# maxjaritz/mvpnet

Hardware: AMD Instinct MI355X
Metric: chunks/sec (8192 pts, 3x160x120 views) fwd+bwd (higher is better)
Workload: dtype f32; 1 GPU; configs[2]: MVPNet lifting (unproject + pixel k-NN + gather) + FeatureAggregation + PN2SSG full train step (fwd+loss+bwd+Adam), 2D CNN replaced by a resident 64-ch feature map; cfg=mvpnet_3d_unet_resnet34_pn2ssg.yaml, chunks_per_gpu=32, points=8192, views=3x160x120, feature_channels=64, k=3, parallelism=dp1 (one process per GPU, 1 grad all-reduce/step), launch=eager, cpu_affinity=32 logical cpus of 256 (0 .. 183)

## Files before the change

include/mvp_hip.h:

```cpp
#ifndef MVP_HIP_H_
#define MVP_HIP_H_

#include <stddef.h>
#include <stdint.h>

#ifdef __cplusplus
extern "C" {
#endif

typedef void* mvp_stream_t;

#define MVP_OK 0
#define MVP_EINVAL (-1)
#define MVP_EUNSUPPORTED (-2)
#define MVP_ENULL (-3)

const char* mvp_version(void);
const char* mvp_strerror(int code);

int mvp_set_fps_mode(int mode);

int mvp_fps_f32(const float* points, int64_t B, int64_t N, int64_t D, int64_t M, int64_t* index, mvp_stream_t stream);
int mvp_fps_f64(const double* points, int64_t B, int64_t N, int64_t D, int64_t M, int64_t* index, mvp_stream_t stream);
int mvp_fps_shape_f32(const float* points, int64_t B, int64_t N, int64_t D, int64_t M, int64_t* index, int shape, mvp_stream_t stream);
// ... 291 lines not shown
                             const float* act_mean, const float* act_invstd, const float* act_gamma, const float* act_beta, float* ymax,
                             float* ymin, uint8_t* amax, uint8_t* amin, double* stat, double* partial, float eps, float momentum,
                             float* mean, float* invstd, float* running_mean, float* running_var, int64_t* num_batches_tracked,
                             mvp_stream_t stream);
int mvp_pool_finalize_f32(const float* ymax, const float* ymin, const uint8_t* amax, const uint8_t* amin, const float* mean,
                          const float* invstd, const float* gamma, const float* beta, int64_t G, int64_t C, int relu, float* out,
                          uint8_t* arg, float* ysel, mvp_stream_t stream);
int mvp_pool_backward_stats_f32(const float* dout, const float* out, const float* ysel, const float* mean, const float* invstd,
                                int64_t G, int64_t C, int relu, double* stat, double* partial, mvp_stream_t stream);
int mvp_mlp_input_grad_f32(const float* dY, int64_t R, int64_t Cout, const float* W, int64_t Cin, const float* y_prev,
                           const float* mean, const float* invstd, const float* gamma, const float* beta, float* dZ,
                           double* stat, double* partial, mvp_stream_t stream);
int mvp_mlp_input_grad_dropout_f32(const float* dY, int64_t R, int64_t Cout, const float* W, int64_t Cin, const float* y_prev,
                                   const float* mean, const float* invstd, const float* gamma, const float* beta, float drop_p,
                                   uint64_t drop_seed, float* dZ, double* stat, double* partial, mvp_stream_t stream);

int64_t mvp_mlp_layer_backward_partial_count(int64_t R, int64_t Cp);
int mvp_mlp_layer_backward_f32(const float* G, const float* Yi, const float* mean_i, const float* invstd_i, const float* gamma_i,
                               const double* stat_i, float* dgamma_i, float* dbeta_i, int training, const float* X, int64_t ldx,
                               const float* act_mean, const float* act_invstd, const float* act_gamma, const float* act_beta,
                               const float* W, int64_t ldw, int64_t R, int64_t C, int64_t Cp, float* dW, int64_t lddw, float* dZ,
                               double* stat_prev, double* partial, const float* pool_dout, const float* pool_out,
                               const uint8_t* pool_arg, mvp_stream_t stream);
int mvp_mlp_layer_backward_ws_f32(const float* G, const float* Yi, const float* mean_i, const float* invstd_i, const float* gamma_i,
                               const double* stat_i, float* dgamma_i, float* dbeta_i, int training, const float* X, int64_t ldx,
                               const float* act_mean, const float* act_invstd, const float* act_gamma, const float* act_beta,
                               const float* W, int64_t ldw, int64_t R, int64_t C, int64_t Cp, float* dW, int64_t lddw, float* dZ,
                               double* stat_prev, double* partial, const float* pool_dout, const float* pool_out,
                               const uint8_t* pool_arg, float* workspace, int64_t workspace_floats, mvp_stream_t stream);
int mvp_mlp_layer_backward_wide_p_f32(const float* G, const float* Yi, const float* mean_i, const float* invstd_i, const float* gamma_i,
// ... 83 lines not shown
    num_batches_tracked, int precision, int precision_backward, mvp_stream_t stream);
int mvp_mlp_forward_rel_bn_p_f32(const float* X, int64_t R, int64_t Cin, int64_t ldx, const float* W, int64_t ldw, int64_t Cout,
    const float* rel, const float* wrel, float* Y, double* stat, double* partial, float eps, float momentum, float* mean, float*
    invstd, float* running_mean, float* running_var, int64_t* num_batches_tracked, int precision, int precision_backward,
    mvp_stream_t stream);
int mvp_mlp_forward_pool_p_f32(const float* X, int64_t R, int64_t Cin, int64_t ldx, const float* W, int64_t ldw, int64_t Cout,
    const float* act_mean, const float* act_invstd, const float* act_gamma, const float* act_beta, float* ymax, float* ymin,
    uint8_t* amax, uint8_t* amin, double* stat, double* partial, float eps, float momentum, float* mean, float* invstd, float*
    running_mean, float* running_var, int64_t* num_batches_tracked, int precision, int precision_backward, mvp_stream_t stream);
int mvp_mlp_input_grad_p_f32(const float* dY, int64_t R, int64_t Cout, const float* W, int64_t Cin, const float* y_prev, const
    float* mean, const float* invstd, const float* gamma, const float* beta, float* dZ, double* stat, double* partial, int
    precision, int precision_backward, mvp_stream_t stream);
int mvp_mlp_input_grad_dropout_p_f32(const float* dY, int64_t R, int64_t Cout, const float* W, int64_t Cin, const float* y_prev, const
    float* mean, const float* invstd, const float* gamma, const float* beta, float drop_p, uint64_t drop_seed, float* dZ, double* stat,
    double* partial, int precision, int precision_backward, mvp_stream_t stream);
int mvp_mlp_weight_grad_p_f32(const float* dY, const float* X, int64_t R, int64_t Cout, int64_t Cin, int64_t ldx, const float*
    act_mean, const float* act_invstd, const float* act_gamma, const float* act_beta, float* dW, int64_t lddw, int precision,
    int precision_backward, mvp_stream_t stream);
int mvp_mlp_weight_grad_ws_p_f32(const float* dY, const float* X, int64_t R, int64_t Cout, int64_t Cin, int64_t ldx, const
    float* act_mean, const float* act_invstd, const float* act_gamma, const float* act_beta, float* dW, int64_t lddw, float*
    workspace, int64_t workspace_floats, int precision, int precision_backward, mvp_stream_t stream);
int mvp_mlp_layer_backward_p_f32(const float* G, const float* Yi, const float* mean_i, const float* invstd_i, const float*
    gamma_i, const double* stat_i, float* dgamma_i, float* dbeta_i, int training, const float* X, int64_t ldx, const float*
    act_mean, const float* act_invstd, const float* act_gamma, const float* act_beta, const float* W, int64_t ldw, int64_t R,
    int64_t C, int64_t Cp, float* dW, int64_t lddw, float* dZ, double* stat_prev, double* partial, const float* pool_dout, const
    float* pool_out, const uint8_t* pool_arg, int precision, int precision_backward, mvp_stream_t stream);
int mvp_mlp_layer_backward_ws_p_f32(const float* G, const float* Yi, const float* mean_i, const float* invstd_i, const float*
    gamma_i, const double* stat_i, float* dgamma_i, float* dbeta_i, int training, const float* X, int64_t ldx, const float*
    act_mean, const float* act_invstd, const float* act_gamma, const float* act_beta, const float* W, int64_t ldw, int64_t R,
    int64_t C, int64_t Cp, float* dW, int64_t lddw, float* dZ, double* stat_prev, double* partial, const float* pool_dout, const
// ... 92 lines not shown
```

mvpnet_amd/csrc/mlp.hip:

```cpp
#include "common.h"
#include "stats_reduce.h"
#include "mlp_common.h"
#include "dropout.h"
#include <algorithm>

int mvp_mlp_stream_forward(const float* X, int64_t R, int Cin, int ldx, const float* W, int ldw, int Cout, const float* act_mean,
                           const float* act_invstd, const float* act_gamma, const float* act_beta, const float* bias, float* Y,
                           double* stat, double* partial, int ns, float bn_eps, float bn_momentum, float* bn_mean, float* bn_invstd,
                           float* bn_running_mean, float* bn_running_var, int64_t* bn_num_batches, float* ymax, float* ymin,
                           uint8_t* amax, uint8_t* amin, hipStream_t s);

int g_mlp_terms = 6;
int g_mlp_terms_bwd = 3;
int g_mlp_min_width = 0;
thread_local int tl_mlp_terms = -1;
thread_local int tl_mlp_terms_bwd = -1;
int g_mlp_stream = 1;

namespace {


constexpr int kMT = 256;
constexpr int kBM = 128;

// ... 613 lines not shown
    for (int i = 0; i < 16; ++i) {
      const int co = co0 + wco + (i & 3) + 8 * (i >> 2) + 4 * (lane >> 5);
#ifdef MVP_EXP_DW_STORE
      if (co < Cout && ci < Cin) *(dW + (size_t)co * lddw + ci) = acc[i];
#else
      if (co < Cout && ci < Cin) atomicAdd(dW + (size_t)co * lddw + ci, acc[i]);
#endif
    }
  }
}

template <int TMB, int TNB, int NS, bool FIN = false, bool REL = false>
__global__ __launch_bounds__(kMT) void mlp_dw_bf_kernel(const float* __restrict__ dY, const float* __restrict__ X, int64_t R,
                                                        int Cout, int Cin, int ldx, InAct act, int64_t rows_per_block,
                                                        float* __restrict__ dW, int lddw, float* __restrict__ ws, DyFinish fin = DyFinish{},
                                                        const float* __restrict__ X2 = nullptr, float* __restrict__ dW2 = nullptr) {
  using SP = SplitPairs<NS>;
  constexpr int NRB = REL ? TMB : 0;
  __shared__ float red[2][(TMB * TNB + NRB) * 16 * 64];
  const int tid = threadIdx.x, lane = tid & 63, wave = tid >> 6;
  const int c = lane & 31, g = lane >> 5;
  const int co0 = blockIdx.x * (32 * TMB), ci0 = blockIdx.y * (32 * TNB);
  const int64_t r_begin = (int64_t)blockIdx.z * rows_per_block;
  const int64_t r_end = min(R, r_begin + rows_per_block);
  f32x16 acc[TMB][TNB];
#pragma unroll
  for (int a = 0; a < TMB; ++a)
#pragma unroll
    for (int b = 0; b < TNB; ++b)
#pragma unroll
      for (int i = 0; i < 16; ++i) acc[a][b][i] = 0.f;
// ... 72 lines not shown
      unsigned q[4][NS];
#pragma unroll
      for (int h2 = 0; h2 < 4; ++h2) split_pair<NS>(v[2 * h2], v[2 * h2 + 1], q[h2]);
#pragma unroll
      for (int pc = 0; pc < NS; ++pc) fa[a][pc] = u32x4{q[0][pc], q[1][pc], q[2][pc], q[3][pc]};
    }
#pragma unroll
    for (int b = 0; b < TNB; ++b) {
      float v[8];
#pragma unroll
      for (int p = 0; p < 8; ++p) {
        float x = xn[b][p];
        if (has_act) {
          const float z = ((x - pm[b]) * pi[b]) * pg[b] + pb[b];
          x = z > 0.f ? z : 0.f;
        }
        v[p] = (rok[p] && xok[b]) ? x : 0.f;
      }
      unsigned q[4][NS];
#pragma unroll
      for (int h2 = 0; h2 < 4; ++h2) split_pair<NS>(v[2 * h2], v[2 * h2 + 1], q[h2]);
#pragma unroll
      for (int pc = 0; pc < NS; ++pc) fb[b][pc] = u32x4{q[0][pc], q[1][pc], q[2][pc], q[3][pc]};
    }
    if constexpr (REL) {
      float v[8];
#pragma unroll
      for (int p = 0; p < 8; ++p) v[p] = (rok[p] && c < 4) ? rn[p] : 0.f;
      unsigned q[4][NS];
#pragma unroll
// ... 350 lines not shown
                         rows_per_block, dW, (int)lddw, w);                                                                        \
    else                                                                                                                           \
      hipLaunchKernelGGL((mlp_dw_kernel<M_, N_, false>), grid, dim3(kMT), 0, s, dY, X, R, (int)Cout, (int)Cin, (int)ldx, act,        \
                         rows_per_block, dW, (int)lddw, w);                                                                        \
    if (w)                                                                                                                         \
      hipLaunchKernelGGL((dw_reduce_kernel<(M_) / 32, (N_) / 32>), dim3((unsigned)(tiles * ((M_) / 32) * ((N_) / 32) * 16)), dim3(256), 0, \
                         s, w, (int)splits, (int)grid.x, (int)grid.y, (int)Cout, (int)Cin, dW, (int)lddw);                         \
  } while (0)
  if (TM == 32 && TN == 32) MVP_DW_LAUNCH(32, 32);
  else if (TM == 32) MVP_DW_LAUNCH(32, 64);
  else if (TN == 32) MVP_DW_LAUNCH(64, 32);
  else MVP_DW_LAUNCH(64, 64);
#undef MVP_DW_LAUNCH
  return mvp_launch_status();
}
}

MVP_API int mvp_mlp_weight_grad_f32(const float* dY, const float* X, int64_t R, int64_t Cout, int64_t Cin, int64_t ldx,
                                    const float* act_mean, const float* act_invstd, const float* act_gamma,
                                    const float* act_beta, float* dW, int64_t lddw, mvp_stream_t stream) {
  return weight_grad_impl(dY, X, R, Cout, Cin, ldx, act_mean, act_invstd, act_gamma, act_beta, dW, lddw, nullptr, 0, stream);
}

MVP_API int64_t mvp_mlp_weight_grad_workspace_floats(void) { return (int64_t)1536 * 4096; }
MVP_API int mvp_mlp_weight_grad_ws_f32(const float* dY, const float* X, int64_t R, int64_t Cout, int64_t Cin, int64_t ldx,
                                       const float* act_mean, const float* act_invstd, const float* act_gamma, const float* act_beta,
                                       float* dW, int64_t lddw, float* workspace, int64_t workspace_floats, mvp_stream_t stream) {
  return weight_grad_impl(dY, X, R, Cout, Cin, ldx, act_mean, act_invstd, act_gamma, act_beta, dW, lddw, workspace, workspace_floats, stream);
}

// ... 157 lines not shown
```

mvpnet_amd/csrc/mlp_prec.hip:

```cpp
#include "mlp_common.h"

namespace {
struct PrecisionArg {
  int old_terms, old_bwd;
  bool ok;
  PrecisionArg(int terms, int bwd) : old_terms(tl_mlp_terms), old_bwd(tl_mlp_terms_bwd) {
    ok = (terms == -1 || terms == 0 || terms == 1 || terms == 3 || terms == 6) && (bwd == -1 || bwd == 1 || bwd == 3 || bwd == 6);
    if (ok && terms >= 0) tl_mlp_terms = terms;
    if (ok && bwd >= 0) tl_mlp_terms_bwd = bwd;
  }
  ~PrecisionArg() {
    tl_mlp_terms = old_terms;
    tl_mlp_terms_bwd = old_bwd;
  }
};
}

#define MVP_WITH_PRECISION(call)             \
  PrecisionArg scope(precision, precision_backward); \
  if (!scope.ok) return MVP_EINVAL;          \
  return call

MVP_API int mvp_mlp_forward_p_f32(const float* X, int64_t R, int64_t Cin, int64_t ldx, const float* W, int64_t ldw, int64_t Cout,
                                  const float* act_mean, const float* act_invstd, const float* act_gamma, const float* act_beta,
// ... 22 lines not shown
                                       float momentum, float* mean, float* invstd, float* running_mean, float* running_var,
                                       int64_t* num_batches_tracked, int precision, int precision_backward, mvp_stream_t stream) {
  MVP_WITH_PRECISION(mvp_mlp_forward_pool_f32(X, R, Cin, ldx, W, ldw, Cout, act_mean, act_invstd, act_gamma, act_beta, ymax, ymin, amax, amin, stat,
                                              partial, eps, momentum, mean, invstd, running_mean, running_var, num_batches_tracked, stream));
}
MVP_API int mvp_mlp_input_grad_p_f32(const float* dY, int64_t R, int64_t Cout, const float* W, int64_t Cin, const float* y_prev,
                                     const float* mean, const float* invstd, const float* gamma, const float* beta, float* dZ, double* stat,
                                     double* partial, int precision, int precision_backward, mvp_stream_t stream) {
  MVP_WITH_PRECISION(mvp_mlp_input_grad_f32(dY, R, Cout, W, Cin, y_prev, mean, invstd, gamma, beta, dZ, stat, partial, stream));
}
MVP_API int mvp_mlp_input_grad_dropout_p_f32(const float* dY, int64_t R, int64_t Cout, const float* W, int64_t Cin, const float* y_prev,
                                             const float* mean, const float* invstd, const float* gamma, const float* beta, float drop_p,
                                             uint64_t drop_seed, float* dZ, double* stat, double* partial, int precision, int precision_backward,
                                             mvp_stream_t stream) {
  MVP_WITH_PRECISION(mvp_mlp_input_grad_dropout_f32(dY, R, Cout, W, Cin, y_prev, mean, invstd, gamma, beta, drop_p, drop_seed, dZ, stat, partial, stream));
}
MVP_API int mvp_mlp_weight_grad_p_f32(const float* dY, const float* X, int64_t R, int64_t Cout, int64_t Cin, int64_t ldx,
                                      const float* act_mean, const float* act_invstd, const float* act_gamma, const float* act_beta,
                                      float* dW, int64_t lddw, int precision, int precision_backward, mvp_stream_t stream) {
  MVP_WITH_PRECISION(mvp_mlp_weight_grad_f32(dY, X, R, Cout, Cin, ldx, act_mean, act_invstd, act_gamma, act_beta, dW, lddw, stream));
}
MVP_API int mvp_mlp_weight_grad_ws_p_f32(const float* dY, const float* X, int64_t R, int64_t Cout, int64_t Cin, int64_t ldx,
                                         const float* act_mean, const float* act_invstd, const float* act_gamma, const float* act_beta,
                                         float* dW, int64_t lddw, float* workspace, int64_t workspace_floats, int precision,
                                         int precision_backward, mvp_stream_t stream) {
  MVP_WITH_PRECISION(mvp_mlp_weight_grad_ws_f32(dY, X, R, Cout, Cin, ldx, act_mean, act_invstd, act_gamma, act_beta, dW, lddw, workspace,
                                                workspace_floats, stream));
}
MVP_API int mvp_mlp_layer_backward_p_f32(const float* G, const float* Yi, const float* mean_i, const float* invstd_i, const float* gamma_i,
                                         const double* stat_i, float* dgamma_i, float* dbeta_i, int training, const float* X, int64_t ldx,
// ... 76 lines not shown
```

mvpnet_amd/csrc/mlp_stream.hip:

```cpp
#include "mlp_common.h"
#include "stats_reduce.h"
#include <algorithm>

namespace {

constexpr int kST = 256;
constexpr int kSLd = 36;

struct StreamArgs {
  const float* X;
  int64_t R;
  int Cin, ldx;
  const float* W;
  int ldw, Cout;
  InAct act;
  const float* bias;
  float* Y;
  double* partial;
  double* stat;
  int finalize;
  BnFinalize fin;
  int64_t tiles_per_wg;
  float* ymax;
  float* ymin;
  uint8_t* amax;
  uint8_t* amin;
};

template <int KS, int NB, bool ACT, int NS, bool POOL>
__global__ __launch_bounds__(kST) void mlp_stream_fwd_kernel(StreamArgs p) {
  using SP = SplitPairs<NS>;
  constexpr int kCols = NB * 32;
  constexpr int kWBytes = KS * NS * kCols * 64;
  __shared__ __attribute__((aligned(16))) unsigned char Wl[kWBytes];
  __shared__ __attribute__((aligned(16))) float Ps[4][KS * 32];
  __shared__ __attribute__((aligned(16))) float tiles[4][32 * kSLd];
  __shared__ double sred[2][4][kCols];
  const int tid = threadIdx.x, lane = tid & 63, wave = tid >> 6;
  const int li = lane & 31, lh = lane >> 5;
  const int Cin = p.Cin, Cout = p.Cout;

  for (int t = tid; t < kCols * KS * 8; t += kST) {
    const int co = t % kCols, kqi = t / kCols;
    const int k = 4 * kqi;
    float v[4];
// ... 41 lines not shown
      for (int tt = 0; tt < 4; ++tt) dst[sl][tt] = *reinterpret_cast<const float4*>(xrow + min(32 * sl + 8 * tt + 4 * lh, Cin - 4));
  };
#pragma unroll
  for (int u = 0; u < PF; ++u)
    if (t_begin + wave + 4 * u < t_end) load_a(an[u], t_begin + wave + 4 * u);
  for (int64_t tb = t_begin + wave; tb < t_end; tb += 4 * PF) {
#pragma unroll
   for (int u = 0; u < PF; ++u) {
    const int64_t t = tb + 4 * u;
    if (t >= t_end) break;
    float4 ac[KS][4];
#pragma unroll
    for (int sl = 0; sl < KS; ++sl)
#pragma unroll
      for (int tt = 0; tt < 4; ++tt) ac[sl][tt] = an[u][sl][tt];
    if (t + 4 * PF < t_end) load_a(an[u], t + 4 * PF);
    f32x16 acc[NB];
#pragma unroll
    for (int j = 0; j < NB; ++j)
#pragma unroll
      for (int i = 0; i < 16; ++i) acc[j][i] = 0.f;
#pragma unroll
    for (int sl = 0; sl < KS; ++sl) {
      float v[4][4];
#pragma unroll
      for (int tt = 0; tt < 4; ++tt) {
        v[tt][0] = ac[sl][tt].x; v[tt][1] = ac[sl][tt].y; v[tt][2] = ac[sl][tt].z; v[tt][3] = ac[sl][tt].w;
        if constexpr (ACT) {
          const int k = 32 * sl + 8 * tt + 4 * lh;
          const float4 m4 = *reinterpret_cast<const float4*>(&Ps[0][k]), i4 = *reinterpret_cast<const float4*>(&Ps[1][k]);
          const float4 g4 = *reinterpret_cast<const float4*>(&Ps[2][k]), b4 = *reinterpret_cast<const float4*>(&Ps[3][k]);
          const float pm[4] = {m4.x, m4.y, m4.z, m4.w}, pi[4] = {i4.x, i4.y, i4.z, i4.w};
          const float pg[4] = {g4.x, g4.y, g4.z, g4.w}, pb[4] = {b4.x, b4.y, b4.z, b4.w};
#pragma unroll
          for (int e = 0; e < 4; ++e) {
            const float a = ((v[tt][e] - pm[e]) * pi[e]) * pg[e] + pb[e];
            v[tt][e] = a > 0.f ? a : 0.f;
          }
        }
      }
#pragma unroll
      for (int s = 0; s < 2; ++s) {
        unsigned q0[NS], q1[NS], q2[NS], q3[NS];
        split_pair<NS>(v[2 * s][0], v[2 * s][1], q0);
        split_pair<NS>(v[2 * s][2], v[2 * s][3], q1);
        split_pair<NS>(v[2 * s + 1][0], v[2 * s + 1][1], q2);
        split_pair<NS>(v[2 * s + 1][2], v[2 * s + 1][3], q3);
        u32x4 af[NS];
#pragma unroll
        for (int pc = 0; pc < NS; ++pc) af[pc] = u32x4{q0[pc], q1[pc], q2[pc], q3[pc]};
        constexpr int JG = NB >= 2 ? 2 : 1;
#pragma unroll
// ... 132 lines not shown
    }
  }
}

template <int KS, int NB, int NS>
void launch_stream(const StreamArgs& a, unsigned grid, bool has_act, hipStream_t s) {
  if (a.ymax) {
    if (has_act) hipLaunchKernelGGL((mlp_stream_fwd_kernel<KS, NB, true, NS, true>), dim3(grid), dim3(kST), 0, s, a);
    else hipLaunchKernelGGL((mlp_stream_fwd_kernel<KS, NB, false, NS, true>), dim3(grid), dim3(kST), 0, s, a);
    return;
  }
  if (has_act) hipLaunchKernelGGL((mlp_stream_fwd_kernel<KS, NB, true, NS, false>), dim3(grid), dim3(kST), 0, s, a);
  else hipLaunchKernelGGL((mlp_stream_fwd_kernel<KS, NB, false, NS, false>), dim3(grid), dim3(kST), 0, s, a);
}

}

int mvp_mlp_stream_forward(const float* X, int64_t R, int Cin, int ldx, const float* W, int ldw, int Cout, const float* act_mean,
                           const float* act_invstd, const float* act_gamma, const float* act_beta, const float* bias, float* Y,
                           double* stat, double* partial, int ns, float bn_eps, float bn_momentum, float* bn_mean, float* bn_invstd,
                           float* bn_running_mean, float* bn_running_var, int64_t* bn_num_batches, float* ymax, float* ymin,
                           uint8_t* amax, uint8_t* amin, hipStream_t s) {
  const InAct act{act_mean, act_invstd, act_gamma, act_beta};
  if (ns == 0 || Cin > 128 || Cout > 128 || Cin < 4 || Cout % 4 != 0 || R < 32768 || (stat && !partial)) return MVP_EUNSUPPORTED;
  if (ldx % 4 != 0 || Cin % 4 != 0 || ((uintptr_t)X % 16) != 0 || (!ymax && ((uintptr_t)Y % 16) != 0)) return MVP_EUNSUPPORTED;
  if (ymax && R % 32 != 0) return MVP_EUNSUPPORTED;
  static const bool tail = []() { const char* e = getenv("MVP_STREAM_TAIL"); return !(e && e[0] == '0'); }();
  StreamArgs a{X, R, Cin, ldx, W, ldw, Cout, act, bias, Y, (stat && !tail) ? partial : nullptr, (stat && tail) ? stat : nullptr, bn_mean ? 1 : 0,
               BnFinalize{R, bn_eps, bn_momentum, bn_mean, bn_invstd, bn_running_mean, bn_running_var, bn_num_batches}, 0, ymax, ymin, amax, amin};
  const int64_t ntiles = cdiv(R, 32);
  const int ks = (int)cdiv(Cin, 32), nb = Cout <= 32 ? 1 : Cout <= 64 ? 2 : 4;
  const int64_t lds = (int64_t)ks * ns * nb * 32 * 64;
  const int64_t per_cu = std::max<int64_t>(1, std::min<int64_t>(4, (140 * 1024) / (lds + 24 * 1024)));
  int64_t wgs = std::min<int64_t>(256 * per_cu, std::min<int64_t>(cdiv(R, 128), cdiv(ntiles, 16)));
  wgs = std::max<int64_t>(wgs, 1);
  a.tiles_per_wg = cdiv(cdiv(ntiles, wgs), 4) * 4;
  const unsigned grid = (unsigned)cdiv(ntiles, a.tiles_per_wg);
  const bool has_act = act.mean != nullptr;
#define MVP_STREAM(KS_, NB_)                                                      \
  do {                                                                            \
    if (ns == 1) launch_stream<KS_, NB_, 1>(a, grid, has_act, s);                  \
    else if (ns == 2) launch_stream<KS_, NB_, 2>(a, grid, has_act, s);             \
    else launch_stream<KS_, NB_, 3>(a, grid, has_act, s);                          \
  } while (0)
#define MVP_STREAM_NB(KS_)                       \
  do {                                           \
    if (nb == 1) MVP_STREAM(KS_, 1);             \
    else if (nb == 2) MVP_STREAM(KS_, 2);        \
    else MVP_STREAM(KS_, 4);                     \
  } while (0)
  switch (ks) {
    case 1: MVP_STREAM_NB(1); break;
    case 2: MVP_STREAM_NB(2); break;
// ... 1 lines not shown
    default: MVP_STREAM_NB(4); break;
  }
#undef MVP_STREAM_NB
#undef MVP_STREAM
  int rc = mvp_launch_status();
  if (rc != MVP_OK) return rc;
  if (a.partial) {
    if (bn_mean)
      launch_stats_reduce_finalize(partial, (int64_t)grid, 2 * Cout, stat,
                                   BnFinalize{R, bn_eps, bn_momentum, bn_mean, bn_invstd, bn_running_mean, bn_running_var, bn_num_batches}, s);
    else
      launch_stats_reduce(partial, (int64_t)grid, 2 * Cout, stat, s);
  }
  return mvp_launch_status();
}
```

mvpnet_amd/pn2.py:

```python
import os

import torch
import torch.nn as nn

from .nn import SharedMLP, SharedMLPDO, batch_index_select, xavier_uniform
from . import ops
from . import rows as R
from . import _lib as L


TRAIN_FPS_SHAPE = int(os.environ.get('MVP_TRAIN_FPS_SHAPE', '1'))
FPS_PREFIX = os.environ.get('MVP_FPS_PREFIX', '1') != '0'
NATIVE_PLAN = os.environ.get('MVP_NATIVE_PLAN', '1') != '0'
MERGE_HEAD = os.environ.get('MVP_MERGE_HEAD', '1') != '0'
HEAD_HANDOVER = os.environ.get('MVP_HEAD_HANDOVER', '1') != '0'


def centroid_levels(xyz, index, counts):
    B, N, D = xyz.shape
    M = index.size(1)
    assert counts[0] == M and all(0 < b <= a for a, b in zip(counts, counts[1:])) and len(counts) <= 8
    if xyz.is_cuda and xyz.dtype == torch.float32:
        import ctypes
        xyz, index = xyz.contiguous(), index.contiguous()
# ... 490 lines not shown
                    if ev is not None:
                        cur.wait_event(ev)
                if level + 1 == len(self.sa_modules) and plan.get('event') is not None:
                    cur.wait_event(plan['event'])
            xyz, feature = sa(xyz, feature, rows=True, geometry=geometry)
            xyzs.append(xyz)
            feats.append(feature)
        up = feats[-1]
        x = None
        hand = None
        head_hand = None
        watched = [_has_hooks(fp) for fp in self.fp_modules]
        for level, fp in enumerate(self.fp_modules):
            geo = None if plan is None else plan['fp'][level]
            if MERGE_HEAD and level + 1 == len(self.fp_modules) and up.is_cuda and not _has_hooks(fp) and not _has_hooks(self.mlp_seg):
                head_hand = R.ActivationHandOver() if (HEAD_HANDOVER and torch.is_grad_enabled() and not _has_hooks(self.seg_logit)) else None
                x = fp(xyzs[-2 - level], xyzs[-1 - level], feats[-2 - level], up, rows=True, geometry=geo, tail=(self.mlp_seg, self.training),
                       sparse_act=hand, act_out=head_hand)
                if x is not None:
                    x = x.reshape(B * N, -1)
                    break
                head_hand = None
            nxt = None
            if (level + 1 < len(self.fp_modules) and up.is_cuda and torch.is_grad_enabled() and not watched[level] and not watched[level + 1]
                    and self.fp_modules[level + 1].interpolator is not None):
                nxt = R.ActivationHandOver()
            up = fp(xyzs[-2 - level], xyzs[-1 - level], feats[-2 - level], up, rows=True, geometry=geo, sparse_act=hand, act_out=nxt)
            hand = nxt
        if x is None:
            up = up.reshape(B * N, -1)
            x = R.shared_mlp_rows(up, self.mlp_seg, dropout_p=self.mlp_seg.p, training=self.training)
# ... 10 lines not shown
```

mvpnet_amd/rows.py:

```python
import os
import weakref

import torch
import torch.nn.functional as F
from torch.autograd.function import once_differentiable

from . import _lib as L


FUSE_BWD_MAX_COUT = int(os.environ.get('MVP_BWD_FUSE_MAXC', '64'))
FUSE_BWD_MAX_CIN = int(os.environ.get('MVP_BWD_FUSE_MAXCIN', '96'))
PARTIAL_MIN_ROWS = int(os.environ.get('MVP_PARTIAL_MIN_ROWS', '65536'))
WIDE_BWD = os.environ.get('MVP_BWD_WIDE', '1') != '0'
WIDE_BWD_MIN_ROWS = int(os.environ.get('MVP_BWD_WIDE_MIN_ROWS', '16384'))


WIDE_BWD_64 = os.environ.get('MVP_BWD_WIDE64', '1') != '0'
WIDE_BWD_POOLED = os.environ.get('MVP_BWD_WIDE_POOLED', '1') != '0'
WIDE_BWD_64_MIN_ROWS = int(os.environ.get('MVP_BWD_WIDE64_MIN_ROWS', '262144'))


DX_WIDE = os.environ.get('MVP_DX_WIDE', '0') == '1'
DX_WIDE_MIN_ROWS = int(os.environ.get('MVP_DX_WIDE_MIN_ROWS', '16384'))
DX_WIDE_MAX_COUT = int(os.environ.get('MVP_DX_WIDE_MAXC', '512'))
# ... 498 lines not shown
        raise RuntimeError('interp_rows: float32 feature with C % 4 == 0 expected')
    return InterpRows.apply(feature.contiguous(), index.contiguous(), weight.contiguous())


class DeferredFinish:
    ENABLED = os.environ.get('MVP_DEFER_FINISH', '1') != '0'
    __slots__ = ('info', 'accepts')

    def __init__(self):
        self.info = None
        self.accepts = False


class ActivationHandOver:
    ENABLED = os.environ.get('MVP_ACT_HANDOVER', '1') != '0'
    __slots__ = ('info', 'stat')

    def __init__(self):
        self.info = None
        self.stat = None


class InterpAddRows(torch.autograd.Function):

    @staticmethod
    def forward(ctx, feature, index, weight, add, want_stat, offsets=None, slots=None, defer=None):
        L.require_gpu(feature, index, weight, add)
        B, N1, C = feature.shape
        N2 = index.size(1)
        dev = feature.device
        out = torch.empty((B, N2, C), dtype=torch.float32, device=dev)
        bn = want_stat if isinstance(want_stat, torch.nn.Module) else None
        stat = zero_pool.zeros(2 * C + (1 if bn is not None else 0), torch.float64, dev) if want_stat else None
        partial = torch.empty(L.lib().mvp_group_lin_partial_count(B, C, N2, 1), dtype=torch.float64, device=dev) if want_stat else None
        mi = torch.empty(2 * C, dtype=torch.float32, device=dev) if bn is not None else None
# ... 277 lines not shown
            st = self.st_arena[self.st_off:self.st_off + 2 * cin]
            self.st_off += 2 * cin
        dz = torch.empty((self.R, cin), dtype=torch.float32, device=self.dev) if need_dz else None
        dgb = torch.empty((2, cout), dtype=torch.float32, device=self.dev) if fin else (None, None)
        return self.dw_arena[off:off + cout * cin].view(cout, cin), st, dz, dgb[0], dgb[1]

    def head(self, g, out, arg):
        ctx, nl, K, R, ys, dev = self.ctx, self.nl, self.K, self.R, self.ys, self.dev
        y, mean, invstd, gamma, beta = self.bn[-1]
        py, pmean, pinvstd, pgamma, pbeta = self.bnp[-1]
        cl, G, training = y.size(1), R // K, int(self.training)
        drop_p, drop_seed = ctx.dropout
        if ctx.act_out is not None and ctx.act_out.stat is not None:
            handed, ctx.act_out.stat = ctx.act_out.stat, None
            return g, handed, None, None
        wl = self.params[3 * (nl - 1)]
        wide = bool(not ctx.pooled and nl >= 2 and wl is not None and g.is_cuda and R * cl < 2 ** 32 and aligned16(g, y, ys[nl - 2]) and
                    wide_backward_ok(self.prec, R, wl.size(0), wl.size(1), ys[nl - 2].size(1)))
        wide_sum = wide and WIDE_BWD_POOLED and K > 1 and arg is None and drop_p == 0
        self.last_wide = wide = wide_sum or (wide and K == 1)
        if not (ctx.pooled or wide or drop_p > 0):
            dy, dgam, dbet = _bn_backward(g, out, arg, y, mean, invstd, gamma, beta, G, K, cl, True, self.training)
            return dy, None, dgam, dbet
        stat = torch.empty(2 * cl, dtype=torch.float64, device=dev)
        if ctx.pooled:
            L.call('mvp_pool_backward_stats_f32', g, L.ptr(g), L.ptr(out), py, pmean, pinvstd, G, cl, 1, L.ptr(stat), L.ptr(_cs_partial(G, cl, dev)))
            self.pool = (g, out, arg)
            return None, stat, None, None
        if wide_sum:
            L.call('mvp_bn_rows_backward_f32', g, L.ptr(g), None, None, py, pmean, pinvstd, pgamma, pbeta, G, K, cl, 1, training, L.ptr(stat),
# ... 82 lines not shown
        dw, stat, dz, dgam, dbet = self.outputs(i, w, need_dz, fin)
        part = torch.empty(L.lib().mvp_mlp_layer_backward_partial_count(R, cin), dtype=torch.float64, device=self.dev) if (i > 0 and need_dz) else None
        pg, po, pa = (None, None, None) if gcur is not None else self.pool
        L.call('mvp_mlp_layer_backward_f32', src, L.ptr(gcur), fy if gcur is not None else None, fm, fi, fg, L.ptr(pending), L.ptr(dgam), L.ptr(dbet),
               int(self.training), L.ptr(src), src.size(1), *(self.bnp[i - 1][1:] if i else _NONE4), L.ptr(w), cin, R, cout, cin, L.ptr(dw), cin, L.ptr(dz),
               L.ptr(stat), L.ptr(part), L.ptr(pg), L.ptr(po), L.ptr(pa), prec=self.prec)
        return dz, stat, dw, dgam, dbet

    def tile(self, i, gcur, w, src, need_dz):
        dw, stat, dz, _, _ = self.outputs(i, w, need_dz)
        self.tile_weight_grad(i, gcur, w, src, dw)
        if need_dz:
            L.call('mvp_mlp_input_grad_f32', gcur, L.ptr(gcur), self.R, w.size(0), L.ptr(w), w.size(1), *(self.bnp[i - 1] if i else (None,) * 5), L.ptr(dz),
                   L.ptr(stat), L.ptr(_partial(self.R, w.size(1), self.dev) if i > 0 else None), prec=self.prec)
        return dz, stat, dw, None, None


class MLPChainRows(torch.autograd.Function):

    @staticmethod
    def forward(ctx, x0, training, K, eps_mom, bn_buffers, first_stat, opts, *params):
        nl = len(params) // 3
        R = x0.size(0)
        dev = x0.device
        prec = ctx.prec = L.current_precision()
        drop_p, drop_seed = opts.get('drop_p', 0.0), opts.get('drop_seed', 0)
        ctx.dw_use = opts.get('use')
        ctx.defer = opts.get('defer')
        pool_sum = bool(opts.get('sum', False))
        rel, w0_param = ctx.rel = opts.get('rel', (None, None))
# ... 14 lines not shown
            if w is None:
                assert i == 0
                y, mean, invstd = _fwd_given(x0, training, first_stat, stat, bn_buffers[i], eps, mom)
            elif i == 0 and rel is not None:
                y, mean, invstd = _fwd_rel(x, rel, w, weight_slices.get(w0_param, x0.size(1), w.size(1), 4), training, stat, bn_buffers[i], eps, mom, prec)
            elif pooled and i == nl - 1:
                y, mean, invstd, out, arg = _fwd_pool(x, w, act, gamma, beta, K, stat, bn_buffers[i], eps, mom, prec)
            else:
                y, mean, invstd = _fwd_layer(x, w, act, training, stat, bn_buffers[i], eps, mom, prec)
            ys.append(y)
            means.append(mean)
            invstds.append(invstd)
            x, act = y, (L.ptr(mean), L.ptr(invstd), L.ptr(gamma), L.ptr(beta))
        cl = ys[-1].size(1)
        G = R // K
        if not pooled and drop_p > 0:
            assert K == 1
            out, arg = torch.empty((R, cl), dtype=torch.float32, device=dev), None
            L.call('mvp_bn_rows_forward_dropout_f32', x0, L.ptr(ys[-1]), L.ptr(params[-2]), L.ptr(params[-1]), R, cl, 0, 0.0, 0.0, 1, None, None,
                   None, L.ptr(means[-1]), L.ptr(invstds[-1]), L.ptr(out), None, float(drop_p), int(drop_seed))
        elif not pooled:
            out, arg = _bn_apply(ys[-1], means[-1], invstds[-1], params[-2], params[-1], G, K, cl, True, pool_sum)
        ao = opts.get('act_out')
        ctx.act_out = None
        if ao is not None and ActivationHandOver.ENABLED and not pooled and K == 1 and training is not None:
            ao.info, ao.stat = (ys[-1], means[-1], invstds[-1], params[-2], params[-1], float(drop_p), int(drop_seed)), None
            ctx.act_out = ao
        ctx.first_linear = params[0] is not None
        ctx.pooled = pooled
        ctx.save_for_backward(x0, out, arg, *ys, *means, *invstds, *[p for p in params if p is not None])
        ctx.cfg = (nl, training, K, R)
        return out

    @staticmethod
    @once_differentiable
    def backward(ctx, grad_out):
        nl, training, K, R = ctx.cfg
        saved = ctx.saved_tensors
        x0, out, arg = saved[0], saved[1], saved[2]
        ys = saved[3:3 + nl]
        params = list(saved[3 + 3 * nl:])
# ... 55 lines not shown
        return g[..., :ctx.C].contiguous(), None, None


def relation_rows(feature, src_xyz, tgt_xyz):
    return RelationRows.apply(feature.contiguous(), src_xyz.contiguous(), tgt_xyz.contiguous())


class LinearRows(torch.autograd.Function):

    @staticmethod
    def forward(ctx, x, w_full, bias, c0=0, c1=None, sink=None, act_src=None):
        ctx.sink = sink
        info = None if act_src is None else act_src.info
        ctx.act_src = act_src if (info is not None and ActivationHandOver.ENABLED and x.is_cuda and tuple(info[0].shape) == tuple(x.shape)) else None
        prec = ctx.prec = L.current_precision()
        w2 = w_full.detach().reshape(w_full.size(0), -1)
        c1 = w2.size(1) if c1 is None else c1
        R, ldx = x.shape
        cin = c1 - c0
        if w2.is_cuda and w2.dtype == torch.float32:
            w = weight_slices.get(w_full, c0, c1, ldx)
        else:
            w = w2[:, c0:c1]
            if ldx != cin:
                w = torch.nn.functional.pad(w, (0, ldx - cin))
            w = w.contiguous()
        L.require_gpu(x, w, bias)
        cout = w.size(0)
        y = torch.empty((R, cout), dtype=torch.float32, device=x.device)
        L.call('mvp_mlp_forward_f32', x, L.ptr(x), R, ldx, ldx, L.ptr(w), ldx, cout, None, None, None, None, L.ptr(bias), L.ptr(y), None, None, prec=prec)
        ctx.save_for_backward(x, w)
        ctx.has_bias = bias is not None
        ctx.slice = (c0, cin, tuple(w_full.shape))
        ctx.bias_param = bias if (bias is not None and bias.is_leaf) else None
        ctx.dw_use = WeightUse([w_full]) if (DW_SIDE_STREAM and LINEAR_ASIDE and sink is None and c0 == 0 and c1 == w2.size(1) and ctx.needs_input_grad[1]) else None
        return y

    @staticmethod
    @once_differentiable
    def backward(ctx, gy):
        x, w = ctx.saved_tensors
        R, cin = x.shape
        cout = w.size(0)
        gy = gy.contiguous()
        gx = gw = gb = None
# ... 12 lines not shown
                    L.call('mvp_mlp_input_grad_f32', gy, L.ptr(gy), R, cout, L.ptr(w), cin, L.ptr(yp), L.ptr(pm), L.ptr(pi), L.ptr(pg), L.ptr(pb), L.ptr(gx),
                           L.ptr(stat), part, prec=ctx.prec)
                src.stat = stat
            else:
                L.call('mvp_mlp_input_grad_f32', gy, L.ptr(gy), R, cout, L.ptr(w), cin, None, None, None, None, None, L.ptr(gx), None, None, prec=ctx.prec)
        if ctx.needs_input_grad[1]:
            c0, ncol, shape = ctx.slice
            sink = ctx.sink
            if sink is not None:
                buf = sink.buffer(gy.device)
                sink.run(gy.device, 'mvp_mlp_weight_grad_f32', (L.ptr(gy), L.ptr(x), R, cout, ncol, cin, None, None, None, None,
                                                                L.ptr_at(buf, c0), sink.numel // cout), (gy, x), prec=ctx.prec)
                gw = sink.done()
            else:
                gw = zero_pool.zeros(shape, torch.float32, w.device)
                wg_args = (L.ptr(gy), L.ptr(x), R, cout, ncol, cin, None, None, None, None, L.ptr_at(gw, c0), gw.numel() // cout)
                use = ctx.dw_use
                aside = use is not None and DW_SIDE_STREAM and use.aside_ok()
                _weight_grad(aside, gy.device, 'mvp_mlp_weight_grad_f32', wg_args, (gy, x), ctx.prec)
                if use is not None:
                    use.done = True
        if ctx.has_bias and ctx.needs_input_grad[2]:
            st = side_stream.streams.get(gy.device)
            bp = ctx.bias_param
            if (aside and st is not None and gy.device in side_stream.open and bp is not None and bp.grad is None and not bp._backward_hooks
                    and not bp._post_accumulate_grad_hooks):
                gb = torch.empty(cout, dtype=gy.dtype, device=gy.device)
                with torch.cuda.stream(st[0]):
                    torch.sum(gy, 0, out=gb)
            else:
                gb = gy.sum(0)
        return gx, gw, gb, None, None, None, None


# ... 278 lines not shown
```

Baseline: 5360 chunks/s.

## Fuse head BN+ReLU+dropout into seg-logit linear forward and weight-grad kernels

The head MLP's final activation (BN apply, ReLU, dropout) is no longer materialised as a separate tensor. The following seg-logit linear reads the raw pre-BN output and applies BN, ReLU and dropout inline in the stream forward kernel and in the dW kernel. New dropout-aware kernel variants and entry points are added, and a lazy hand-over flag falls back to materialising the activation when the fused conditions do not hold. This removes one full R×C write and read pass plus a kernel launch, at the cost of recomputing the dropout hash in two kernels and more fragile coupling between the modules.

```diff
diff --git a/include/mvp_hip.h b/include/mvp_hip.h
--- a/include/mvp_hip.h
+++ b/include/mvp_hip.h
@@ -329,6 +329,13 @@
 int mvp_mlp_input_grad_dropout_f32(const float* dY, int64_t R, int64_t Cout, const float* W, int64_t Cin, const float* y_prev,
                                    const float* mean, const float* invstd, const float* gamma, const float* beta, float drop_p,
                                    uint64_t drop_seed, float* dZ, double* stat, double* partial, mvp_stream_t stream);
+int mvp_mlp_forward_dropout_ok(int64_t R, int64_t Cin, int64_t Cout);
+int mvp_mlp_forward_dropout_f32(const float* X, int64_t R, int64_t Cin, const float* W, int64_t ldw, int64_t Cout, const float* act_mean,
+                                const float* act_invstd, const float* act_gamma, const float* act_beta, float drop_p, uint64_t drop_seed,
+                                const float* bias, float* Y, mvp_stream_t stream);
+int mvp_mlp_weight_grad_dropout_f32(const float* dY, const float* X, int64_t R, int64_t Cout, int64_t Cin, const float* act_mean,
+                                    const float* act_invstd, const float* act_gamma, const float* act_beta, float drop_p, uint64_t drop_seed,
+                                    float* dW, int64_t lddw, mvp_stream_t stream);
 
 int64_t mvp_mlp_layer_backward_partial_count(int64_t R, int64_t Cp);
 int mvp_mlp_layer_backward_f32(const float* G, const float* Yi, const float* mean_i, const float* invstd_i, const float* gamma_i,
@@ -442,6 +449,12 @@
 int mvp_mlp_input_grad_dropout_p_f32(const float* dY, int64_t R, int64_t Cout, const float* W, int64_t Cin, const float* y_prev, const
     float* mean, const float* invstd, const float* gamma, const float* beta, float drop_p, uint64_t drop_seed, float* dZ, double* stat,
     double* partial, int precision, int precision_backward, mvp_stream_t stream);
+int mvp_mlp_forward_dropout_p_f32(const float* X, int64_t R, int64_t Cin, const float* W, int64_t ldw, int64_t Cout, const float* act_mean,
+    const float* act_invstd, const float* act_gamma, const float* act_beta, float drop_p, uint64_t drop_seed, const float* bias, float* Y,
+    int precision, int precision_backward, mvp_stream_t stream);
+int mvp_mlp_weight_grad_dropout_p_f32(const float* dY, const float* X, int64_t R, int64_t Cout, int64_t Cin, const float* act_mean,
+    const float* act_invstd, const float* act_gamma, const float* act_beta, float drop_p, uint64_t drop_seed, float* dW, int64_t lddw,
+    int precision, int precision_backward, mvp_stream_t stream);
 int mvp_mlp_weight_grad_p_f32(const float* dY, const float* X, int64_t R, int64_t Cout, int64_t Cin, int64_t ldx, const float*
     act_mean, const float* act_invstd, const float* act_gamma, const float* act_beta, float* dW, int64_t lddw, int precision,
     int precision_backward, mvp_stream_t stream);
diff --git a/mvpnet_amd/csrc/mlp.hip b/mvpnet_amd/csrc/mlp.hip
--- a/mvpnet_amd/csrc/mlp.hip
+++ b/mvpnet_amd/csrc/mlp.hip
@@ -651,7 +651,9 @@
 __global__ __launch_bounds__(kMT) void mlp_dw_bf_kernel(const float* __restrict__ dY, const float* __restrict__ X, int64_t R,
                                                         int Cout, int Cin, int ldx, InAct act, int64_t rows_per_block,
                                                         float* __restrict__ dW, int lddw, float* __restrict__ ws, DyFinish fin = DyFinish{},
-                                                        const float* __restrict__ X2 = nullptr, float* __restrict__ dW2 = nullptr) {
+                                                        const float* __restrict__ X2 = nullptr, float* __restrict__ dW2 = nullptr,
+                                                        Dropout drop = Dropout{0u, 0u, 1.0f}) {
+  constexpr bool DROP = TMB == 1 && TNB == 2 && !FIN && !REL;
   using SP = SplitPairs<NS>;
   constexpr int NRB = REL ? TMB : 0;
   __shared__ float red[2][(TMB * TNB + NRB) * 16 * 64];
@@ -754,6 +756,9 @@
         if (has_act) {
           const float z = ((x - pm[b]) * pi[b]) * pg[b] + pb[b];
           x = z > 0.f ? z : 0.f;
+        }
+        if constexpr (DROP) {
+          if (drop.thresh) x *= drop.factor((unsigned)(min(r0 + 8 * g + p, R - 1) * Cin + xcol[b]));
         }
         v[p] = (rok[p] && xok[b]) ? x : 0.f;
       }
@@ -1134,6 +1139,41 @@
 #undef MVP_DW_LAUNCH
   return mvp_launch_status();
 }
+}
+
+MVP_API int mvp_mlp_weight_grad_dropout_f32(const float* dY, const float* X, int64_t R, int64_t Cout, int64_t Cin, const float* act_mean,
+                                            const float* act_invstd, const float* act_gamma, const float* act_beta, float drop_p,
+                                            uint64_t drop_seed, float* dW, int64_t lddw, mvp_stream_t stream) {
+  MVP_NONNULL(dY);
+  MVP_NONNULL(X);
+  MVP_NONNULL(dW);
+  MVP_NONNULL(act_mean);
+  MVP_NONNULL(act_invstd);
+  MVP_NONNULL(act_gamma);
+  MVP_NONNULL(act_beta);
+  MVP_REQUIRE(R > 0 && Cin > 0 && Cout > 0 && Cin < (1 << 20) && lddw >= Cin && lddw < (1 << 24));
+  const int ns = std::max(Cin, Cout) >= g_mlp_min_width ? mlp_bwd_pieces() : 0;
+  if (ns == 0 || Cout > 32 || Cin <= 32) return MVP_EUNSUPPORTED;
+  Dropout drop;
+  const int rc = make_dropout(drop_p, drop_seed, R, Cin, 1, &drop);
+  if (rc != MVP_OK) return rc;
+  hipStream_t s = static_cast<hipStream_t>(stream);
+  const int64_t tiles = cdiv(Cin, 64);
+  static const int64_t wg_target = []() { const char* e = getenv("MVP_DW_WORKGROUPS"); return e ? (int64_t)atoi(e) : (int64_t)1024; }();
+  int64_t splits = std::min<int64_t>(cdiv(wg_target, tiles), 512);
+  int64_t rows_per_block = cdiv(cdiv(R, splits), 64) * 64;
+  if (rows_per_block < 256) rows_per_block = 256;
+  splits = cdiv(R, rows_per_block);
+  const InAct act{act_mean, act_invstd, act_gamma, act_beta};
+  const dim3 grid(1, (unsigned)tiles, (unsigned)splits);
+#define MVP_DWBF_DROP(NS_)                                                                                                                    \
+  hipLaunchKernelGGL((mlp_dw_bf_kernel<1, 2, NS_>), grid, dim3(kMT), 0, s, dY, X, R, (int)Cout, (int)Cin, (int)Cin, act, rows_per_block, dW, \
+                     (int)lddw, (float*)nullptr, DyFinish{}, (const float*)nullptr, (float*)nullptr, drop)
+  if (ns == 1) MVP_DWBF_DROP(1);
+  else if (ns == 2) MVP_DWBF_DROP(2);
+  else MVP_DWBF_DROP(3);
+#undef MVP_DWBF_DROP
+  return mvp_launch_status();
 }
 
 MVP_API int mvp_mlp_weight_grad_f32(const float* dY, const float* X, int64_t R, int64_t Cout, int64_t Cin, int64_t ldx,
diff --git a/mvpnet_amd/csrc/mlp_prec.hip b/mvpnet_amd/csrc/mlp_prec.hip
--- a/mvpnet_amd/csrc/mlp_prec.hip
+++ b/mvpnet_amd/csrc/mlp_prec.hip
@@ -60,6 +60,17 @@
                                              uint64_t drop_seed, float* dZ, double* stat, double* partial, int precision, int precision_backward,
                                              mvp_stream_t stream) {
   MVP_WITH_PRECISION(mvp_mlp_input_grad_dropout_f32(dY, R, Cout, W, Cin, y_prev, mean, invstd, gamma, beta, drop_p, drop_seed, dZ, stat, partial, stream));
+}
+MVP_API int mvp_mlp_forward_dropout_p_f32(const float* X, int64_t R, int64_t Cin, const float* W, int64_t ldw, int64_t Cout, const float* act_mean,
+                                          const float* act_invstd, const float* act_gamma, const float* act_beta, float drop_p, uint64_t drop_seed,
+                                          const float* bias, float* Y, int precision, int precision_backward, mvp_stream_t stream) {
+  MVP_WITH_PRECISION(mvp_mlp_forward_dropout_f32(X, R, Cin, W, ldw, Cout, act_mean, act_invstd, act_gamma, act_beta, drop_p, drop_seed, bias, Y, stream));
+}
+MVP_API int mvp_mlp_weight_grad_dropout_p_f32(const float* dY, const float* X, int64_t R, int64_t Cout, int64_t Cin, const float* act_mean,
+                                              const float* act_invstd, const float* act_gamma, const float* act_beta, float drop_p,
+                                              uint64_t drop_seed, float* dW, int64_t lddw, int precision, int precision_backward,
+                                              mvp_stream_t stream) {
+  MVP_WITH_PRECISION(mvp_mlp_weight_grad_dropout_f32(dY, X, R, Cout, Cin, act_mean, act_invstd, act_gamma, act_beta, drop_p, drop_seed, dW, lddw, stream));
 }
 MVP_API int mvp_mlp_weight_grad_p_f32(const float* dY, const float* X, int64_t R, int64_t Cout, int64_t Cin, int64_t ldx,
                                       const float* act_mean, const float* act_invstd, const float* act_gamma, const float* act_beta,
diff --git a/mvpnet_amd/csrc/mlp_stream.hip b/mvpnet_amd/csrc/mlp_stream.hip
--- a/mvpnet_amd/csrc/mlp_stream.hip
+++ b/mvpnet_amd/csrc/mlp_stream.hip
@@ -1,5 +1,6 @@
 #include "mlp_common.h"
 #include "stats_reduce.h"
+#include "dropout.h"
 #include <algorithm>
 
 namespace {
@@ -25,10 +26,12 @@
   float* ymin;
   uint8_t* amax;
   uint8_t* amin;
+  Dropout drop;
 };
 
 template <int KS, int NB, bool ACT, int NS, bool POOL>
 __global__ __launch_bounds__(kST) void mlp_stream_fwd_kernel(StreamArgs p) {
+  constexpr bool DROP = ACT && !POOL && KS == 4 && NB == 1;
   using SP = SplitPairs<NS>;
   constexpr int kCols = NB * 32;
   constexpr int kWBytes = KS * NS * kCols * 64;
@@ -100,6 +103,7 @@
     for (int sl = 0; sl < KS; ++sl)
 #pragma unroll
       for (int tt = 0; tt < 4; ++tt) ac[sl][tt] = an[u][sl][tt];
+    const unsigned erow = DROP ? (unsigned)(min(t * 32 + li, p.R - 1) * Cin) : 0u;
     if (t + 4 * PF < t_end) load_a(an[u], t + 4 * PF);
     f32x16 acc[NB];
 #pragma unroll
@@ -122,6 +126,13 @@
           for (int e = 0; e < 4; ++e) {
             const float a = ((v[tt][e] - pm[e]) * pi[e]) * pg[e] + pb[e];
             v[tt][e] = a > 0.f ? a : 0.f;
+          }
+          if constexpr (DROP) {
+            if (p.drop.thresh) {
+              const unsigned e0 = erow + (unsigned)min(k, Cin - 4);
+#pragma unroll
+              for (int e = 0; e < 4; ++e) v[tt][e] *= p.drop.factor(e0 + e);
+            }
           }
         }
       }
@@ -284,6 +295,12 @@
   else hipLaunchKernelGGL((mlp_stream_fwd_kernel<KS, NB, false, NS, false>), dim3(grid), dim3(kST), 0, s, a);
 }
 
+int stream_forward_impl(const float* X, int64_t R, int Cin, int ldx, const float* W, int ldw, int Cout, const float* act_mean,
+                        const float* act_invstd, const float* act_gamma, const float* act_beta, const float* bias, float* Y, double* stat,
+                        double* partial, int ns, float bn_eps, float bn_momentum, float* bn_mean, float* bn_invstd, float* bn_running_mean,
+                        float* bn_running_var, int64_t* bn_num_batches, float* ymax, float* ymin, uint8_t* amax, uint8_t* amin,
+                        const Dropout* drop, hipStream_t s);
+
 }
 
 int mvp_mlp_stream_forward(const float* X, int64_t R, int Cin, int ldx, const float* W, int ldw, int Cout, const float* act_mean,
@@ -291,13 +308,25 @@
                            double* stat, double* partial, int ns, float bn_eps, float bn_momentum, float* bn_mean, float* bn_invstd,
                            float* bn_running_mean, float* bn_running_var, int64_t* bn_num_batches, float* ymax, float* ymin,
                            uint8_t* amax, uint8_t* amin, hipStream_t s) {
+  return stream_forward_impl(X, R, Cin, ldx, W, ldw, Cout, act_mean, act_invstd, act_gamma, act_beta, bias, Y, stat, partial, ns, bn_eps, bn_momentum,
+                             bn_mean, bn_invstd, bn_running_mean, bn_running_var, bn_num_batches, ymax, ymin, amax, amin, nullptr, s);
+}
+
+namespace {
+
+int stream_forward_impl(const float* X, int64_t R, int Cin, int ldx, const float* W, int ldw, int Cout, const float* act_mean,
+                        const float* act_invstd, const float* act_gamma, const float* act_beta, const float* bias, float* Y, double* stat,
+                        double* partial, int ns, float bn_eps, float bn_momentum, float* bn_mean, float* bn_invstd, float* bn_running_mean,
+                        float* bn_running_var, int64_t* bn_num_batches, float* ymax, float* ymin, uint8_t* amax, uint8_t* amin,
+                        const Dropout* drop, hipStream_t s) {
   const InAct act{act_mean, act_invstd, act_gamma, act_beta};
   if (ns == 0 || Cin > 128 || Cout > 128 || Cin < 4 || Cout % 4 != 0 || R < 32768 || (stat && !partial)) return MVP_EUNSUPPORTED;
   if (ldx % 4 != 0 || Cin % 4 != 0 || ((uintptr_t)X % 16) != 0 || (!ymax && ((uintptr_t)Y % 16) != 0)) return MVP_EUNSUPPORTED;
   if (ymax && R % 32 != 0) return MVP_EUNSUPPORTED;
   static const bool tail = []() { const char* e = getenv("MVP_STREAM_TAIL"); return !(e && e[0] == '0'); }();
   StreamArgs a{X, R, Cin, ldx, W, ldw, Cout, act, bias, Y, (stat && !tail) ? partial : nullptr, (stat && tail) ? stat : nullptr, bn_mean ? 1 : 0,
-               BnFinalize{R, bn_eps, bn_momentum, bn_mean, bn_invstd, bn_running_mean, bn_running_var, bn_num_batches}, 0, ymax, ymin, amax, amin};
+               BnFinalize{R, bn_eps, bn_momentum, bn_mean, bn_invstd, bn_running_mean, bn_running_var, bn_num_batches}, 0, ymax, ymin, amax, amin,
+               drop ? *drop : Dropout{0u, 0u, 1.0f}};
   const int64_t ntiles = cdiv(R, 32);
   const int ks = (int)cdiv(Cin, 32), nb = Cout <= 32 ? 1 : Cout <= 64 ? 2 : 4;
   const int64_t lds = (int64_t)ks * ns * nb * 32 * 64;
@@ -307,6 +336,9 @@
   a.tiles_per_wg = cdiv(cdiv(ntiles, wgs), 4) * 4;
   const unsigned grid = (unsigned)cdiv(ntiles, a.tiles_per_wg);
   const bool has_act = act.mean != nullptr;
+  if (drop) {
+    if (ks != 4 || nb != 1 || !has_act || ymax || ldx != Cin) return MVP_EUNSUPPORTED;
+  }
 #define MVP_STREAM(KS_, NB_)                                                      \
   do {                                                                            \
     if (ns == 1) launch_stream<KS_, NB_, 1>(a, grid, has_act, s);                  \
@@ -338,3 +370,33 @@
   }
   return mvp_launch_status();
 }
+
+}
+
+extern int g_mlp_min_width;
+extern int g_mlp_stream;
+
+MVP_API int mvp_mlp_forward_dropout_ok(int64_t R, int64_t Cin, int64_t Cout) {
+  return (g_mlp_stream && mlp_fwd_pieces() != 0 && std::max(Cin, Cout) >= g_mlp_min_width && R >= 32768 && R * Cin < (1ll << 32) && Cin > 96 &&
+          Cin <= 128 && Cin % 4 == 0 && Cout >= 4 && Cout <= 32 && Cout % 4 == 0) ? 1 : 0;
+}
+
+MVP_API int mvp_mlp_forward_dropout_f32(const float* X, int64_t R, int64_t Cin, const float* W, int64_t ldw, int64_t Cout, const float* act_mean,
+                                        const float* act_invstd, const float* act_gamma, const float* act_beta, float drop_p, uint64_t drop_seed,
+                                        const float* bias, float* Y, mvp_stream_t stream) {
+  MVP_NONNULL(X);
+  MVP_NONNULL(W);
+  MVP_NONNULL(Y);
+  MVP_NONNULL(act_mean);
+  MVP_NONNULL(act_invstd);
+  MVP_NONNULL(act_gamma);
+  MVP_NONNULL(act_beta);
+  MVP_REQUIRE(R > 0 && Cin > 0 && Cout > 0 && ldw >= Cin);
+  if (!mvp_mlp_forward_dropout_ok(R, Cin, Cout)) return MVP_EUNSUPPORTED;
+  Dropout drop;
+  const int rc = make_dropout(drop_p, drop_seed, R, Cin, 1, &drop);
+  if (rc != MVP_OK) return rc;
+  return stream_forward_impl(X, R, (int)Cin, (int)Cin, W, (int)ldw, (int)Cout, act_mean, act_invstd, act_gamma, act_beta, bias, Y, nullptr, nullptr,
+                             mlp_fwd_pieces(), 0.f, 0.f, nullptr, nullptr, nullptr, nullptr, nullptr, nullptr, nullptr, nullptr, nullptr, &drop,
+                             static_cast<hipStream_t>(stream));
+}
diff --git a/mvpnet_amd/pn2.py b/mvpnet_amd/pn2.py
--- a/mvpnet_amd/pn2.py
+++ b/mvpnet_amd/pn2.py
@@ -528,7 +528,8 @@
         for level, fp in enumerate(self.fp_modules):
             geo = None if plan is None else plan['fp'][level]
             if MERGE_HEAD and level + 1 == len(self.fp_modules) and up.is_cuda and not _has_hooks(fp) and not _has_hooks(self.mlp_seg):
-                head_hand = R.ActivationHandOver() if (HEAD_HANDOVER and torch.is_grad_enabled() and not _has_hooks(self.seg_logit)) else None
+                head_hand = R.ActivationHandOver(lazy_cout=self.num_classes) if (HEAD_HANDOVER and torch.is_grad_enabled() and
+                                                                                  not _has_hooks(self.seg_logit)) else None
                 x = fp(xyzs[-2 - level], xyzs[-1 - level], feats[-2 - level], up, rows=True, geometry=geo, tail=(self.mlp_seg, self.training),
                        sparse_act=hand, act_out=head_hand)
                 if x is not None:
diff --git a/mvpnet_amd/rows.py b/mvpnet_amd/rows.py
--- a/mvpnet_amd/rows.py
+++ b/mvpnet_amd/rows.py
@@ -536,11 +536,14 @@
 
 class ActivationHandOver:
     ENABLED = os.environ.get('MVP_ACT_HANDOVER', '1') != '0'
-    __slots__ = ('info', 'stat')
-
-    def __init__(self):
+    HEAD_TAIL = os.environ.get('MVP_HEAD_TAIL', '1') != '0'
+    __slots__ = ('info', 'stat', 'lazy_cout', 'lazy')
+
+    def __init__(self, lazy_cout=0):
         self.info = None
         self.stat = None
+        self.lazy_cout = int(lazy_cout)
+        self.lazy = False
 
 
 class InterpAddRows(torch.autograd.Function):
@@ -848,6 +851,8 @@
         if ctx.act_out is not None and ctx.act_out.stat is not None:
             handed, ctx.act_out.stat = ctx.act_out.stat, None
             return g, handed, None, None
+        if ctx.lazy_out:
+            raise RuntimeError('MLPChainRows: the output was handed over unmaterialised (ActivationHandOver.lazy) and its consumer left no column sums')
         wl = self.params[3 * (nl - 1)]
         wide = bool(not ctx.pooled and nl >= 2 and wl is not None and g.is_cuda and R * cl < 2 ** 32 and aligned16(g, y, ys[nl - 2]) and
                     wide_backward_ok(self.prec, R, wl.size(0), wl.size(1), ys[nl - 2].size(1)))
@@ -960,6 +965,14 @@
             L.call('mvp_mlp_input_grad_f32', gcur, L.ptr(gcur), self.R, w.size(0), L.ptr(w), w.size(1), *(self.bnp[i - 1] if i else (None,) * 5), L.ptr(dz),
                    L.ptr(stat), L.ptr(_partial(self.R, w.size(1), self.dev) if i > 0 else None), prec=self.prec)
         return dz, stat, dw, None, None
+
+
+def _head_activation(y, mean, invstd, gamma, beta, drop_p, drop_seed):
+    R, cl = y.shape
+    out = torch.empty((R, cl), dtype=torch.float32, device=y.device)
+    L.call('mvp_bn_rows_forward_dropout_f32', y, L.ptr(y), L.ptr(gamma), L.ptr(beta), R, cl, 0, 0.0, 0.0, 1, None, None,
+           None, L.ptr(mean), L.ptr(invstd), L.ptr(out), None, float(drop_p), int(drop_seed))
+    return out
 
 
 class MLPChainRows(torch.autograd.Function):
@@ -1004,17 +1017,21 @@
             x, act = y, (L.ptr(mean), L.ptr(invstd), L.ptr(gamma), L.ptr(beta))
         cl = ys[-1].size(1)
         G = R // K
-        if not pooled and drop_p > 0:
+        ao = opts.get('act_out')
+        hand = ao is not None and ActivationHandOver.ENABLED and not pooled and K == 1 and training is not None
+        lazy = ctx.lazy_out = bool(hand and ao.lazy_cout > 0 and ActivationHandOver.HEAD_TAIL and training and not L.DW_WORKSPACE and x0.is_cuda and
+                                   ys[-1].is_contiguous() and L.lib().mvp_mlp_forward_dropout_ok(R, cl, ao.lazy_cout))
+        if lazy:
+            out, arg = ys[-1], None
+        elif not pooled and drop_p > 0:
             assert K == 1
-            out, arg = torch.empty((R, cl), dtype=torch.float32, device=dev), None
-            L.call('mvp_bn_rows_forward_dropout_f32', x0, L.ptr(ys[-1]), L.ptr(params[-2]), L.ptr(params[-1]), R, cl, 0, 0.0, 0.0, 1, None, None,
-                   None, L.ptr(means[-1]), L.ptr(invstds[-1]), L.ptr(out), None, float(drop_p), int(drop_seed))
+            out, arg = _head_activation(ys[-1], means[-1], invstds[-1], params[-2], params[-1], drop_p, drop_seed), None
         elif not pooled:
             out, arg = _bn_apply(ys[-1], means[-1], invstds[-1], params[-2], params[-1], G, K, cl, True, pool_sum)
-        ao = opts.get('act_out')
         ctx.act_out = None
-        if ao is not None and ActivationHandOver.ENABLED and not pooled and K == 1 and training is not None:
+        if hand:
             ao.info, ao.stat = (ys[-1], means[-1], invstds[-1], params[-2], params[-1], float(drop_p), int(drop_seed)), None
+            ao.lazy = lazy
             ctx.act_out = ao
         ctx.first_linear = params[0] is not None
         ctx.pooled = pooled
@@ -1100,6 +1117,13 @@
         info = None if act_src is None else act_src.info
         ctx.act_src = act_src if (info is not None and ActivationHandOver.ENABLED and x.is_cuda and tuple(info[0].shape) == tuple(x.shape)) else None
         prec = ctx.prec = L.current_precision()
+        lazy = ctx.lazy = bool(act_src is not None and act_src.lazy and ctx.act_src is not None and x.data_ptr() == info[0].data_ptr() and sink is None and
+                               c0 == 0 and (c1 is None or c1 == x.size(1)) and w_full.is_cuda and w_full.dtype == torch.float32 and
+                               w_full.numel() == w_full.size(0) * x.size(1) and w_full.size(0) == act_src.lazy_cout and
+                               L.lib().mvp_mlp_forward_dropout_ok(x.size(0), x.size(1), w_full.size(0)))
+        if act_src is not None and act_src.lazy and not lazy:
+            x = _head_activation(*info)
+            act_src.lazy = False
         w2 = w_full.detach().reshape(w_full.size(0), -1)
         c1 = w2.size(1) if c1 is None else c1
         R, ldx = x.shape
@@ -1114,7 +1138,12 @@
         L.require_gpu(x, w, bias)
         cout = w.size(0)
         y = torch.empty((R, cout), dtype=torch.float32, device=x.device)
-        L.call('mvp_mlp_forward_f32', x, L.ptr(x), R, ldx, ldx, L.ptr(w), ldx, cout, None, None, None, None, L.ptr(bias), L.ptr(y), None, None, prec=prec)
+        if lazy:
+            yp, pm, pi, pg, pb, drop_p, drop_seed = info
+            L.call('mvp_mlp_forward_dropout_f32', x, L.ptr(yp), R, ldx, L.ptr(w), ldx, cout, L.ptr(pm), L.ptr(pi), L.ptr(pg), L.ptr(pb), drop_p, drop_seed,
+                   L.ptr(bias), L.ptr(y), prec=prec)
+        else:
+            L.call('mvp_mlp_forward_f32', x, L.ptr(x), R, ldx, ldx, L.ptr(w), ldx, cout, None, None, None, None, L.ptr(bias), L.ptr(y), None, None, prec=prec)
         ctx.save_for_backward(x, w)
         ctx.has_bias = bias is not None
         ctx.slice = (c0, cin, tuple(w_full.shape))
@@ -1157,10 +1186,19 @@
                 gw = sink.done()
             else:
                 gw = zero_pool.zeros(shape, torch.float32, w.device)
-                wg_args = (L.ptr(gy), L.ptr(x), R, cout, ncol, cin, None, None, None, None, L.ptr_at(gw, c0), gw.numel() // cout)
+                wg_name, wg_args, wg_keep = 'mvp_mlp_weight_grad_f32', (L.ptr(gy), L.ptr(x), R, cout, ncol, cin, None, None, None, None, L.ptr_at(gw, c0),
+                                                                       gw.numel() // cout), (gy, x)
+                if ctx.lazy:
+                    yp, pm, pi, pg, pb, drop_p, drop_seed = ctx.act_src.info
+                    wg_keep = (gy, x, pm, pi, pg, pb)
+                    if drop_p > 0:
+                        wg_name, wg_args = 'mvp_mlp_weight_grad_dropout_f32', (L.ptr(gy), L.ptr(x), R, cout, ncol, L.ptr(pm), L.ptr(pi), L.ptr(pg), L.ptr(pb),
+                                                                              drop_p, drop_seed, L.ptr_at(gw, c0), gw.numel() // cout)
+                    else:
+                        wg_args = wg_args[:6] + (L.ptr(pm), L.ptr(pi), L.ptr(pg), L.ptr(pb)) + wg_args[10:]
                 use = ctx.dw_use
                 aside = use is not None and DW_SIDE_STREAM and use.aside_ok()
-                _weight_grad(aside, gy.device, 'mvp_mlp_weight_grad_f32', wg_args, (gy, x), ctx.prec)
+                _weight_grad(aside, gy.device, wg_name, wg_args, wg_keep, ctx.prec)
                 if use is not None:
                     use.done = True
         if ctx.has_bias and ctx.needs_input_grad[2]:
```

New measurement: 5357 chunks/s. No clear change (-0.1%).
